# atsuki-ichikawa/KoeMorph

Measured on AMD Instinct MI355X. Metric: blendshape frames/sec (52-coef, 256-win, d_model=256), higher is better.
Workload: dtype f32; 1 GPU; C2: 256 windows/GPU x 136448 samples (8.5 s @16 kHz) -> 1024-pt STFT, hop 533, 80-bin log-mel (257 frames) -> dual-stream attention d_model=256, 8 heads, window 256 -> 52 coefficients + EMA; from audio resident in HBM (rotating batches); windows_per_gpu=256, samples_per_window=136448, parallelism=window-sharded x1, no collective

## Files before the change

### koemorph_amd/csrc/km_device.h

```cpp
#pragma once

#include <hip/hip_runtime.h>

#include "koemorph.h"

namespace km {

struct LogParams {
    int log_mode;
    float amin, top_db, db_add, db_scale, log_eps;
};

__device__ __forceinline__ float clamp_lo(float x, float lo) { return __builtin_amdgcn_fmed3f(x, lo, __builtin_inff()); }
__device__ __forceinline__ float db10(float s, float amin) {
    return 3.01029995663981195f * __builtin_amdgcn_logf(clamp_lo(s, amin));
}

__device__ __forceinline__ void log_window_consts(const LogParams& p, float ref, float& ref_db, float& floor_db) {
    ref_db = db10(ref, p.amin);
    floor_db = (db10(ref, p.amin) - ref_db) - p.top_db;
}

__device__ __forceinline__ float db_finish(const LogParams& p, float dbs, float ref_db, float floor_db) {
    float v = dbs - ref_db;
    v = clamp_lo(v, floor_db);
    return (v + p.db_add) * p.db_scale;
}
__device__ __forceinline__ float db_fast_c1(const LogParams& p, float ref_db) { return (p.db_add - ref_db) * p.db_scale; }
__device__ __forceinline__ float db_finish_fast(float dbs, float scale, float c1) { return fmaxf(fmaf(dbs, scale, c1), 0.f); }
struct DbXform { LogParams lp; const unsigned* ref_bits; };

struct LnXform { const float* stats; const float* gamma; const float* beta; int npart; float eps; };
__device__ __forceinline__ void ln_combine(const float2* __restrict__ st, int npart, float eps, float& rs, float& nmurs, float* mean_out = nullptr) {
    float msum = 0.f;
    for (int p = 0; p < npart; ++p) msum += st[p].x;
    const float mean = msum / (float)npart;
    float m2 = 0.f;
    for (int p = 0; p < npart; ++p) { const float dm = st[p].x - mean; m2 += st[p].y + 32.0f * dm * dm; }
    rs = 1.0f / sqrtf(m2 / (float)(32 * npart) + eps);
    nmurs = -mean * rs;
    if (mean_out) *mean_out = mean;
}
__device__ __forceinline__ void ln_combine8(const float2 (&st)[8], int npart, float eps, float& rs, float& nmurs) {
    float msum = 0.f;
#pragma unroll
    for (int p = 0; p < 8; ++p) msum += p < npart ? st[p].x : 0.f;
    const float mean = msum / (float)npart;
    float m2 = 0.f;
#pragma unroll
    for (int p = 0; p < 8; ++p) { const float dm = st[p].x - mean; m2 += p < npart ? st[p].y + 32.0f * dm * dm : 0.f; }
    rs = 1.0f / sqrtf(m2 / (float)(32 * npart) + eps);
    nmurs = -mean * rs;
}
__device__ __forceinline__ float ln_apply(float x, float rs, float nmurs, float gam, float bet) { return fmaf(fmaf(x, rs, nmurs), gam, bet); }

template <int MODE>
__device__ __forceinline__ float log_one_t(const LogParams& p, float s, float ref_db, float floor_db) {
    if (MODE == KM_LOG_LN_EPS) return 0.693147180559945309f * __builtin_amdgcn_logf(s + p.log_eps);
    float v = db10(s, p.amin) - ref_db;
    v = clamp_lo(v, floor_db);
    return (v + p.db_add) * p.db_scale;
}

__device__ __forceinline__ float log_one(const LogParams& p, float s, float ref_db, float floor_db) {
    return p.log_mode == KM_LOG_LN_EPS ? log_one_t<KM_LOG_LN_EPS>(p, s, ref_db, floor_db)
                                       : log_one_t<KM_LOG_DB_MAX>(p, s, ref_db, floor_db);
}

template <int MODE>
__device__ __forceinline__ float4 log_four_t(const LogParams& p, float4 v, float ref_db, float floor_db) {
    return make_float4(log_one_t<MODE>(p, v.x, ref_db, floor_db), log_one_t<MODE>(p, v.y, ref_db, floor_db),
                       log_one_t<MODE>(p, v.z, ref_db, floor_db), log_one_t<MODE>(p, v.w, ref_db, floor_db));
}

__device__ __forceinline__ float row16_sum(float v) {
    v += __int_as_float(__builtin_amdgcn_update_dpp(0, __float_as_int(v), 0xB1, 0xF, 0xF, true));
    v += __int_as_float(__builtin_amdgcn_update_dpp(0, __float_as_int(v), 0x4E, 0xF, 0xF, true));
    v += __int_as_float(__builtin_amdgcn_update_dpp(0, __float_as_int(v), 0x141, 0xF, 0xF, true));
    v += __int_as_float(__builtin_amdgcn_update_dpp(0, __float_as_int(v), 0x140, 0xF, 0xF, true));
    return v;
}

struct EmoArgs {
    const float* emo = nullptr;
    int ED = 0;
    const float *wee_t = nullptr , *bee = nullptr, *lg = nullptr, *lb = nullptr, *we2 = nullptr, *be2 = nullptr,
                *w2 = nullptr, *b2 = nullptr;
    float* zemo = nullptr;
    int d = 256, DH = 128;
};

__device__ __forceinline__ void emotion_window_d256(const EmoArgs& e, int64_t b, float* scratch) {
    constexpr int d = 256, DH = 128;
    float* emo_s = scratch;
    float* e1 = scratch + 256;
    float* part = scratch + 512;
    const int tid = threadIdx.x, lane = tid & 63;
    if (tid < 256) emo_s[tid] = tid < e.ED ? e.emo[b * e.ED + tid] : 0.f;
    __syncthreads();
    {
        const int n = tid & 255, h = __builtin_amdgcn_readfirstlane(tid >> 8);
#pragma unroll 1
        for (int q = 2 * h; q < 2 * h + 2; ++q) {
            const float* wp = e.wee_t + (size_t)64 * q * d + n;
            float w[64];
#pragma unroll
            for (int u = 0; u < 64; ++u) w[u] = wp[u * d];
            float acc = 0.f;
#pragma unroll
            for (int u = 0; u < 64; u += 4) {
                const float4 x = *reinterpret_cast<const float4*>(emo_s + 64 * q + u);
                acc = fmaf(x.x, w[u], acc);
                acc = fmaf(x.y, w[u + 1], acc);
                acc = fmaf(x.z, w[u + 2], acc);
                acc = fmaf(x.w, w[u + 3], acc);
            }
            part[q * d + n] = acc;
        }
    }
    __syncthreads();
    if (tid < 256) {
        float s = e.bee[tid];
#pragma unroll
        for (int q = 0; q < 4; ++q) s += part[q * d + tid];
        e1[tid] = s;
    }
    __syncthreads();
    if (tid < 64) {
        float x[4], s = 0.f;
#pragma unroll
        for (int i = 0; i < 4; ++i) { x[i] = e1[lane + 64 * i]; s += x[i]; }
#pragma unroll
        for (int o = 32; o > 0; o >>= 1) s += __shfl_xor(s, o);
        const float mean = s * (1.0f / d);
        float v = 0.f;
#pragma unroll
        for (int i = 0; i < 4; ++i) { const float t = x[i] - mean; v += t * t; }
#pragma unroll
        for (int o = 32; o > 0; o >>= 1) v += __shfl_xor(v, o);
        const float rstd = 1.0f / sqrtf(v * (1.0f / d) + 1e-5f);
#pragma unroll
        for (int i = 0; i < 4; ++i) {
            const int c = lane + 64 * i;
            e1[c] = (x[i] - mean) * rstd * e.lg[c] + e.lb[c];
        }
    }
    __syncthreads();
    {
        const int m = tid & 127, h = tid >> 7;
#pragma unroll 1
        for (int q = 2 * h; q < 2 * h + 2; ++q) {
            const float* wp = e.we2 + (size_t)32 * q * DH + m;
            float w[32];
#pragma unroll
            for (int u = 0; u < 32; ++u) w[u] = wp[u * DH];
            float acc = 0.f;
#pragma unroll
            for (int u = 0; u < 32; u += 4) {
                const float4 x = *reinterpret_cast<const float4*>(e1 + 32 * q + u);
                acc = fmaf(x.x, w[u], acc);
                acc = fmaf(x.y, w[u + 1], acc);
                acc = fmaf(x.z, w[u + 2], acc);
                acc = fmaf(x.w, w[u + 3], acc);
            }
            part[q * DH + m] = acc;
        }
    }
    __syncthreads();
    if (tid < 64) {
        float s = 0.f;
#pragma unroll
        for (int i = 0; i < 2; ++i) {
            const int mm = lane + 64 * i;
            float hsum = e.be2[mm];
#pragma unroll
            for (int q = 0; q < 8; ++q) hsum += part[q * DH + mm];
            s += fmaxf(hsum, 0.f) * e.w2[mm];
        }
#pragma unroll
        for (int o = 32; o > 0; o >>= 1) s += __shfl_xor(s, o);
        if (lane == 0) e.zemo[b] = s + e.b2[0];
    }
    __syncthreads();
}

struct EmoShape { int d = 0, DH = 0; };

__device__ __forceinline__ void emotion_layer_f4(const float* __restrict__ w, int K, int N, const float* x, float* part) {
    const int tid = threadIdx.x;
    const int tpr = N >> 2;
    const int G = 512 / tpr;
    const int c4 = tid & (tpr - 1), g = tid / tpr;
    const int kc = (K + G - 1) / G;
    const int k0 = g * kc, k1 = (k0 + kc) < K ? (k0 + kc) : K;
    float4 acc = make_float4(0.f, 0.f, 0.f, 0.f);
    const float* wp = w + 4 * c4;
    for (int k = k0; k < k1; k += 16) {
        float4 wv[16];
#pragma unroll
        for (int u = 0; u < 16; ++u) wv[u] = (k + u) < k1 ? *reinterpret_cast<const float4*>(wp + (size_t)(k + u) * N) : make_float4(0.f, 0.f, 0.f, 0.f);
#pragma unroll
        for (int u = 0; u < 16; ++u) {
            const float xv = (k + u) < k1 ? x[k + u] : 0.f;
            acc.x = fmaf(xv, wv[u].x, acc.x); acc.y = fmaf(xv, wv[u].y, acc.y);
            acc.z = fmaf(xv, wv[u].z, acc.z); acc.w = fmaf(xv, wv[u].w, acc.w);
        }
    }
    *reinterpret_cast<float4*>(part + g * N + 4 * c4) = acc;
}

__device__ __forceinline__ void emotion_window_generic(const EmoArgs& e, const EmoShape sh, int64_t b, float* scratch) {
    const int d = sh.d, DH = sh.DH;
    float* emo_s = scratch;
    float* e1 = scratch + 256;
    float* part = e1 + d;
    const int tid = threadIdx.x, lane = tid & 63;
    if (tid < 256) emo_s[tid] = tid < e.ED ? e.emo[b * e.ED + tid] : 0.f;
    __syncthreads();
    emotion_layer_f4(e.wee_t, e.ED, d, emo_s, part);
    __syncthreads();
    {
        const int G1 = 2048 / d;
        for (int n = tid; n < d; n += 512) {
            float s = e.bee[n];
            for (int g = 0; g < G1; ++g) s += part[g * d + n];
            e1[n] = s;
        }
    }
    __syncthreads();
    if (tid < 64) {
        float s = 0.f;
        for (int n = lane; n < d; n += 64) s += e1[n];
#pragma unroll
        for (int o = 32; o > 0; o >>= 1) s += __shfl_xor(s, o);
        const float mean = s / d;
        float v = 0.f;
        for (int n = lane; n < d; n += 64) { const float t = e1[n] - mean; v += t * t; }
#pragma unroll
        for (int o = 32; o > 0; o >>= 1) v += __shfl_xor(v, o);
        const float rstd = 1.0f / sqrtf(v / d + 1e-5f);
        for (int n = lane; n < d; n += 64) e1[n] = (e1[n] - mean) * rstd * e.lg[n] + e.lb[n];
    }
    __syncthreads();
    emotion_layer_f4(e.we2, d, DH, e1, part);
    __syncthreads();
    if (tid < 64) {
        const int G2 = 2048 / DH;
        float s = 0.f;
        for (int m = lane; m < DH; m += 64) {
            float h = e.be2[m];
            for (int g = 0; g < G2; ++g) h += part[g * DH + m];
            s += fmaxf(h, 0.f) * e.w2[m];
        }
#pragma unroll
        for (int o = 32; o > 0; o >>= 1) s += __shfl_xor(s, o);
        if (lane == 0) e.zemo[b] = s + e.b2[0];
    }
    __syncthreads();
}

}
```

### koemorph_amd/csrc/km_mel.hip

```cpp
#include <hip/hip_runtime.h>

#include <cstdlib>

#include "km_context.h"
#include "km_device.h"

namespace km {

#define HIP_TRY(expr)                                                                         \
    do {                                                                                      \
        hipError_t e_ = (expr);                                                               \
        if (e_ != hipSuccess) return fail(KM_ERR_HIP, "%s: %s", #expr, hipGetErrorString(e_)); \
    } while (0)

namespace mel {
constexpr int FPB = 16;
constexpr int WAVES = 4;
constexpr int FFT_BUF = 1152;
}

__device__ __forceinline__ float2 cadd(float2 a, float2 b) { return make_float2(a.x + b.x, a.y + b.y); }
__device__ __forceinline__ float2 csub(float2 a, float2 b) { return make_float2(a.x - b.x, a.y - b.y); }
__device__ __forceinline__ float2 cmul(float2 a, float2 b) {
    return make_float2(a.x * b.x - a.y * b.y, a.x * b.y + a.y * b.x);
// ... 430 lines not shown
#define KM_MEL_W2 0
#endif
__device__ __forceinline__ void swap_lane32(v2f& a, v2f& b) {
    const auto r0 = __builtin_amdgcn_permlane32_swap(__float_as_uint(a.x), __float_as_uint(b.x), false, false);
    const auto r1 = __builtin_amdgcn_permlane32_swap(__float_as_uint(a.y), __float_as_uint(b.y), false, false);
    a = v2f{__uint_as_float(r0[0]), __uint_as_float(r1[0])}; b = v2f{__uint_as_float(r0[1]), __uint_as_float(r1[1])};
}
__device__ __forceinline__ void swap_lane16(v2f& a, v2f& b) {
    const auto r0 = __builtin_amdgcn_permlane16_swap(__float_as_uint(a.x), __float_as_uint(b.x), false, false);
    const auto r1 = __builtin_amdgcn_permlane16_swap(__float_as_uint(a.y), __float_as_uint(b.y), false, false);
    a = v2f{__uint_as_float(r0[0]), __uint_as_float(r1[0])}; b = v2f{__uint_as_float(r0[1]), __uint_as_float(r1[1])};
}
#define KM_XM " row_mask:0xf bank_mask:"
#define KM_XBANK(CT, MT, CA, MA, MB)                                      \
    "s_nop 1\n\t"                                                        \
    "v_mov_b32_dpp %[t0], %[a0] " CT KM_XM MT "\n\t"                      \
    "v_mov_b32_dpp %[t1], %[a1] " CT KM_XM MT "\n\t"                      \
    "v_mov_b32_dpp %[t2], %[a2] " CT KM_XM MT "\n\t"                      \
    "v_mov_b32_dpp %[t3], %[a3] " CT KM_XM MT "\n\t"                      \
    "v_mov_b32_dpp %[a0], %[b0] " CA KM_XM MA "\n\t"                      \
    "v_mov_b32_dpp %[a1], %[b1] " CA KM_XM MA "\n\t"                      \
    "v_mov_b32_dpp %[a2], %[b2] " CA KM_XM MA "\n\t"                      \
    "v_mov_b32_dpp %[a3], %[b3] " CA KM_XM MA "\n\t"                      \
    "v_mov_b32_dpp %[b0], %[t0] quad_perm:[0,1,2,3]" KM_XM MB "\n\t"      \
    "v_mov_b32_dpp %[b1], %[t1] quad_perm:[0,1,2,3]" KM_XM MB "\n\t"      \
    "v_mov_b32_dpp %[b2], %[t2] quad_perm:[0,1,2,3]" KM_XM MB "\n\t"      \
    "v_mov_b32_dpp %[b3], %[t3] quad_perm:[0,1,2,3]" KM_XM MB "\n\t"      \
    "s_nop 0"
#define KM_XBANK_OPERANDS                                                                                              \
    : [t0] "=&v"(t0), [t1] "=&v"(t1), [t2] "=&v"(t2), [t3] "=&v"(t3), [a0] "+v"(p0), [a1] "+v"(p1), [a2] "+v"(p2), [a3] "+v"(p3), \
      [b0] "+v"(q0), [b1] "+v"(q1), [b2] "+v"(q2), [b3] "+v"(q3)
#define KM_XQUAD(QP)                                                       \
    "s_nop 1\n\t"                                                          \
    "v_mov_b32_dpp %[t0], %[a0] " QP KM_XM "0xf\n\t"                        \
    "v_mov_b32_dpp %[t1], %[a1] " QP KM_XM "0xf\n\t"                        \
    "v_mov_b32_dpp %[u0], %[b0] " QP KM_XM "0xf\n\t"                        \
    "v_mov_b32_dpp %[u1], %[b1] " QP KM_XM "0xf\n\t"                        \
    "v_mov_b32_dpp %[t2], %[a2] " QP KM_XM "0xf\n\t"                        \
    "v_mov_b32_dpp %[t3], %[a3] " QP KM_XM "0xf\n\t"                        \
    "v_mov_b32_dpp %[u2], %[b2] " QP KM_XM "0xf\n\t"                        \
    "v_mov_b32_dpp %[u3], %[b3] " QP KM_XM "0xf\n\t"                        \
    "v_cndmask_b32_e64 %[a0], %[a0], %[u0], %[mk]\n\t"                      \
    "v_cndmask_b32_e64 %[a1], %[a1], %[u1], %[mk]\n\t"                      \
    "v_cndmask_b32_e64 %[b0], %[t0], %[b0], %[mk]\n\t"                      \
    "v_cndmask_b32_e64 %[b1], %[t1], %[b1], %[mk]\n\t"                      \
    "v_cndmask_b32_e64 %[a2], %[a2], %[u2], %[mk]\n\t"                      \
    "v_cndmask_b32_e64 %[a3], %[a3], %[u3], %[mk]\n\t"                      \
    "v_cndmask_b32_e64 %[b2], %[t2], %[b2], %[mk]\n\t"                      \
    "v_cndmask_b32_e64 %[b3], %[t3], %[b3], %[mk]\n\t"                      \
    "s_nop 0"
#define KM_XQUAD_OPERANDS                                                                                              \
    : [t0] "=&v"(t0), [t1] "=&v"(t1), [t2] "=&v"(t2), [t3] "=&v"(t3), [u0] "=&v"(u0), [u1] "=&v"(u1), [u2] "=&v"(u2), [u3] "=&v"(u3), \
      [a0] "+v"(p0), [a1] "+v"(p1), [a2] "+v"(p2), [a3] "+v"(p3), [b0] "+v"(q0), [b1] "+v"(q1), [b2] "+v"(q2), [b3] "+v"(q3)       \
    : [mk] "s"(mk)
template <int B>
__device__ __forceinline__ void swap_lane_dpp(v2f& a0, v2f& b0, v2f& a1, v2f& b1) {
    float p0 = a0.x, p1 = a0.y, p2 = a1.x, p3 = a1.y, q0 = b0.x, q1 = b0.y, q2 = b1.x, q3 = b1.y, t0, t1, t2, t3;
    if constexpr (B == 3) KM_ASM(KM_XBANK("row_ror:8", "0xf", "row_ror:8", "0xc", "0x3") KM_XBANK_OPERANDS);
    else if constexpr (B == 2) KM_ASM(KM_XBANK("row_shl:4", "0x5", "row_shr:4", "0xa", "0x5") KM_XBANK_OPERANDS);
    else {
        constexpr unsigned long long mk = B == 1 ? 0xCCCCCCCCCCCCCCCCull : 0xAAAAAAAAAAAAAAAAull;
        float u0, u1, u2, u3;
        if constexpr (B == 1) KM_ASM(KM_XQUAD("quad_perm:[2,3,0,1]") KM_XQUAD_OPERANDS);
        else KM_ASM(KM_XQUAD("quad_perm:[1,0,3,2]") KM_XQUAD_OPERANDS);
    }
    a0 = v2f{p0, p1}; a1 = v2f{p2, p3}; b0 = v2f{q0, q1}; b1 = v2f{q2, q3};
}
__device__ __forceinline__ void exchange_hi(v2f (&y)[8]) {
#pragma unroll
    for (int r = 0; r < 4; ++r) swap_lane32(y[r], y[r + 4]);
#pragma unroll
    for (int r = 0; r < 8; r += 4) { swap_lane16(y[r], y[r + 2]); swap_lane16(y[r + 1], y[r + 3]); }
    swap_lane_dpp<3>(y[0], y[1], y[2], y[3]);
    swap_lane_dpp<3>(y[4], y[5], y[6], y[7]);
}
__device__ __forceinline__ void exchange_lo(v2f (&y)[8]) {
    swap_lane_dpp<2>(y[0], y[4], y[1], y[5]);
    swap_lane_dpp<2>(y[2], y[6], y[3], y[7]);
    swap_lane_dpp<1>(y[0], y[2], y[1], y[3]);
    swap_lane_dpp<1>(y[4], y[6], y[5], y[7]);
    swap_lane_dpp<0>(y[0], y[1], y[2], y[3]);
    swap_lane_dpp<0>(y[4], y[5], y[6], y[7]);
}
__host__ __device__ constexpr int fft_lane_k0(int lane) { return (KM_MEL_XCHG & 1) ? bitrev(lane >> 3, 3) : lane >> 3; }
__host__ __device__ constexpr int fft_lane_bin(int lane) {
    return (KM_MEL_XCHG & 2) ? fft_lane_k0(lane) + 8 * bitrev(lane & 7, 3) : lane;
}
__host__ __device__ constexpr int fft_bin_lane(int c) {
    return (KM_MEL_XCHG & 2) ? 8 * ((KM_MEL_XCHG & 1) ? bitrev(c & 7, 3) : (c & 7)) + bitrev(c >> 3, 3) : c;
}
}

template <bool RING>
__device__ __forceinline__ bool load_frame_rp_fast(const float* __restrict__ x, int Li, int rs, int hop, int f, int lane,
                                                   melrp::v2f (&z)[8]) {
    const int lo = f * hop - 512;
    if (lo < 0 || lo + 1024 > Li) return false;
    int start = lo;
    if constexpr (RING) {
        start += rs;
        start -= start >= Li ? Li : 0;
        if (start + 1024 > Li) return false;
    }
    const float* xp = x + start + 2 * lane;
#pragma unroll
    for (int i = 0; i < 8; ++i) z[i] = melrp::v2f{xp[128 * i], xp[128 * i + 1]};
    return true;
}

__device__ __noinline__ void load_frame_rp_slow(const float* __restrict__ x, int Li, int rs, int ring, int hop, int refl, int f,
                                                int lane, float2* __restrict__ buf) {
    const int p0 = f * hop - 512 + 2 * lane;
    for (int i = 0; i < 8; ++i) {
        float v[2];
        for (int e = 0; e < 2; ++e) {
            int q = p0 + 128 * i + e;
            bool ok = true;
            if (refl) q = q < 0 ? -q : (q >= Li ? 2 * (Li - 1) - q : q);
            else ok = q >= 0 && q < Li;
            if (ring) { q += rs; q -= q >= Li ? Li : 0; }
            v[e] = ok ? x[ok ? q : 0] : 0.f;
        }
        buf[lane + 64 * i] = make_float2(v[0], v[1]);
    }
}

__device__ __forceinline__ int mel_slot_of_lane(int lane) {
    const int m = lane & 31;
    const bool g0 = m < 4 || (m >= 12 && m < 16) || (m >= 20 && m < 28);
    return 2 * (lane >> 5) + (g0 ? 0 : 1);
}
__device__ __forceinline__ int mel_frame_of_lane(int lane) {
    const int m = lane & 31;
    if (m < 4) return m;
    if (m < 12) return m - 4;
    if (m < 16) return m - 8;
    if (m < 20) return m - 8;
    if (m < 28) return m - 12;
    return m - 16;
}
__device__ __forceinline__ int mel_lane_of(int slot, int frame) {
    int m;
    if (slot & 1) m = frame < 8 ? frame + 4 : (frame < 12 ? frame + 8 : frame + 16);
    else m = frame < 4 ? frame : (frame < 8 ? frame + 8 : frame + 12);
    return 32 * (slot >> 1) + m;
}

template <bool RING, bool PACK = false>
__global__ __launch_bounds__(512, 4) void mel_power_rp_kernel(MelArgs a) {
    using namespace melrp;
    extern __shared__ __attribute__((aligned(16))) float smem[];
    float2* fbuf = reinterpret_cast<float2*>(smem);
    float* pw = smem + WAVES * FFT_BUF * 2;
    float* redmax = pw + FPB * NFS;
    int* sched = reinterpret_cast<int*>(redmax + WAVES);
    float* fbw = redmax + WAVES + 4;

#ifdef KM_MEL_STAMP
    const unsigned long long st_entry = __builtin_readcyclecounter(), st_entry_rt = __builtin_amdgcn_s_memrealtime();
#endif
    const int tid = threadIdx.x, lane = tid & 63;
    const int wave = __builtin_amdgcn_readfirstlane(tid >> 6);
#if KM_MEL_REMAP
    const unsigned lin_ = blockIdx.x + gridDim.x * blockIdx.y;
    const int b = (int)(lin_ % gridDim.y), bx = (int)(lin_ / gridDim.y);
#else
    const int b = blockIdx.y, bx = (int)blockIdx.x;
#endif
    const int64_t gw = a.win0 + b;
    const int64_t clip = gw / a.wins_per_clip, woff = (gw - clip * a.wins_per_clip) * a.win_step;
    const float* x = a.audio + clip * a.clip_len + woff;
    const int Lv = (int)((a.clip_len - woff) < a.L ? (a.clip_len - woff) : a.L);
    if (a.ready && !a.ready[b]) return;
    const int rs = RING ? a.ring_start[b] : -1;
    v2f* buf = reinterpret_cast<v2f*>(fbuf + wave * FFT_BUF);
    const int n_chunks = (a.n_frames + FPB - 1) / FPB;
    const unsigned rd2 = lds_offset(buf + (lane >> 3) * 72 + (lane & 7)), rd3 = lds_offset(buf + lane * 9);
    const unsigned wr3 = lds_offset(buf + fft_lane_k0(lane) * 9 + (lane & 7));
    const int cbin = fft_lane_bin(lane);

    v2f zn[8];
    bool zn_ok = false;
    const int fmul = a.frame_mul;
    auto first_frame = [&]() {
        if (KM_MEL_SKIP & 8) {
#pragma unroll
            for (int i = 0; i < 8; ++i) zn[i] = v2f{0.001f * lane, 0.5f + i};
            zn_ok = true;
        } else if (bx * FPB + wave < a.n_frames) zn_ok = load_frame_rp_fast<RING>(x, Lv, rs, a.hop, (bx * FPB + wave) * fmul, lane, zn);
    };
    if (!(KM_MEL_SKIP & 16) && a.emo.emo && bx == (int)gridDim.x - 1) {
        if (a.emo.d == 256 && a.emo.DH == 128) emotion_window_d256(a.emo, gw, pw);
        else emotion_window_generic(a.emo, EmoShape{a.emo.d, a.emo.DH}, gw, pw);
        first_frame();
    } else {
        first_frame();
    }

    const unsigned ctr_last = (unsigned)n_chunks - 1u;
    for (int i = tid; i < a.fbg_nw; i += NT) fbw[i] = a.fbg_weight[i];
    for (int i = tid; i < FPB * (NFS - 513); i += NT) pw[(i / (NFS - 513)) * NFS + 513 + i % (NFS - 513)] = 0.f;

    const int n2 = lane & 7, k0 = fft_lane_k0(lane);
    v2f win2[8], tw1[8], tw2[8], twp[4];
#pragma unroll
    for (int i = 0; i < 8; ++i) {
        win2[i] = v2f{a.window[2 * (lane + 64 * i)], a.window[2 * (lane + 64 * i) + 1]};
        tw1[i] = ld2(a.twiddle + ((2 * lane * bitrev(i, 3)) & 1023));
        tw2[i] = ld2(a.twiddle + ((16 * n2 * bitrev(i, 3)) & 1023));
    }
#pragma unroll
    for (int i = 0; i < 4; ++i) twp[i] = ld2(a.twiddle + cbin + 64 * i);

    int my_gid[NGW];
#pragma unroll
    for (int i = 0; i < NGW; ++i) my_gid[i] = __builtin_amdgcn_readfirstlane(a.fbg_gid[wave * NGW + i]);
    const int* my_desc_p = a.fbg_desc + wave * NGW * 4 + mel_slot_of_lane(lane);
#pragma unroll
    for (int i = 0; i < 8; ++i) asm volatile("" ::"v"(win2[i]), "v"(tw1[i]), "v"(tw2[i]));
#pragma unroll
    for (int i = 0; i < 4; ++i) asm volatile("" ::"v"(twp[i]));
#pragma unroll
    for (int i = 0; i < NGW; ++i) asm volatile("" ::"s"(my_gid[i]));

    float vmax = 0.f;
    int chunk = bx, chunk_next = bx + (int)gridDim.x;
#if defined(KM_MEL_DELAY)
    if (bx & 1) { for (int i = 0; i < KM_MEL_DELAY; i += 16) __builtin_amdgcn_s_sleep(16); }
#endif
#ifdef KM_MEL_STAMP
    unsigned st_acc[16] = {0};
    unsigned long long st_last = __builtin_readcyclecounter();
    const unsigned long long st_first = st_last;
#endif
    while (chunk < n_chunks) {
        unsigned req = 0;
        if (tid == 0) req = atomicAdd(a.chunk_ctr + b, 1u);
        const int f0 = chunk * FPB;
#pragma unroll 1
        for (int pi = 0; pi < FPB / WAVES; ++pi) {
            const int fl = wave + WAVES * pi;
            const int f = f0 + fl;
            if (f < a.n_frames) {
                if (!zn_ok) {
                    load_frame_rp_slow(x, Lv, rs, RING ? 1 : 0, a.hop, a.pad_mode == KM_PAD_REFLECT ? 1 : 0, f * fmul, lane,
                                       reinterpret_cast<float2*>(buf));
                    __builtin_amdgcn_wave_barrier();
#pragma unroll
                    for (int i = 0; i < 8; ++i) zn[i] = buf[lane + 64 * i];
                    __builtin_amdgcn_wave_barrier();
                }
                KM_STAMP(0);
                v2f z[8];
#pragma unroll
                for (int i = 0; i < 8; ++i) z[i] = zn[i] * win2[i];
                if (!(KM_MEL_SKIP & 4)) { dif8(z); cmul7(z, tw1); }
                KM_STAMP(1);
                v2f y[8];
                if ((KM_MEL_XCHG & 1) && !(KM_MEL_SKIP & 2)) {
                    exchange_hi(z);
#pragma unroll
                    for (int i = 0; i < 8; ++i) y[i] = z[i];
                } else if (!(KM_MEL_SKIP & 2)) {
#pragma unroll
                    for (int i = 0; i < 8; ++i) buf[bitrev(i, 3) * 72 + lane] = z[i];
                    __builtin_amdgcn_wave_barrier();
                }
                {
                    const int fnext = pi + 1 < FPB / WAVES ? f + WAVES : chunk_next * FPB + wave;
                    if (!(KM_MEL_SKIP & 8)) zn_ok = fnext < a.n_frames && load_frame_rp_fast<RING>(x, Lv, rs, a.hop, fnext * fmul, lane, zn);
                }
                if (!(KM_MEL_XCHG & 1) && !(KM_MEL_SKIP & 2)) {
                    lds_read8<64>(rd2, y);
                    __builtin_amdgcn_wave_barrier();
                } else if (KM_MEL_SKIP & 2) {
#pragma unroll
                    for (int i = 0; i < 8; ++i) y[i] = z[i];
                }
                KM_STAMP(2);
                if (!(KM_MEL_SKIP & 4)) { dif8(y); cmul7(y, tw2); }
                KM_STAMP(3);
                if ((KM_MEL_XCHG & 2) && !(KM_MEL_SKIP & 2)) {
                    exchange_lo(y);
                } else if (!(KM_MEL_SKIP & 2)) {
#if KM_MEL_W2
#pragma unroll
                    for (int i = 0; i < 8; ++i) buf[(k0 + 8 * bitrev(i, 3)) * 9 + n2] = y[i];
#else
                    lds_write8_bitrev<8 * 9 * 8>(wr3, y);
#endif
                    __builtin_amdgcn_wave_barrier();
                    lds_read8<8>(rd3, y);
                    __builtin_amdgcn_wave_barrier();
                }
                KM_STAMP(4);
                if (!(KM_MEL_SKIP & 4)) dif8(y);
                KM_STAMP(5);
                float* pwr = pw + fl * NFS;
                v2f zk[4], zc[4];
                v2f zmid = y[1];
                if (!(KM_MEL_SKIP & 2)) {
                    const int src = fft_bin_lane((64 - cbin) & 63) << 2;
                    auto perm = [&](v2f v) {
                        return v2f{__int_as_float(__builtin_amdgcn_ds_bpermute(src, __float_as_int(v.x))),
                                   __int_as_float(__builtin_amdgcn_ds_bpermute(src, __float_as_int(v.y)))};
                    };
                    const v2f p7 = perm(y[7]), p3 = perm(y[3]), p5 = perm(y[5]), p1 = perm(y[1]);
                    const bool l0 = lane == 0;
                    zk[0] = y[0]; zk[1] = y[4]; zk[2] = y[2]; zk[3] = y[6];
                    zc[0] = l0 ? y[0] : p7; zc[1] = l0 ? y[7] : p3; zc[2] = l0 ? y[3] : p5; zc[3] = l0 ? y[5] : p1;
                } else {
#pragma unroll
                    for (int i = 0; i < 4; ++i) { zk[i] = y[i]; zc[i] = y[i + 4]; }
                }
                KM_STAMP(6);
                if (!(KM_MEL_SKIP & 4)) post4(zk, zc, twp);
#pragma unroll
                for (int i = 0; i < 4; ++i) {
                    pwr[cbin + 64 * i] = zk[i].x;
                    pwr[2 * 256 - cbin - 64 * i] = zk[i].y;
                }
                if (lane == 0) pwr[256] = 4.0f * (zmid.x * zmid.x + zmid.y * zmid.y);
                KM_STAMP(7);
            }
        }
        KM_STAMP(8);
        int my_desc[NGW];
#pragma unroll
        for (int i = 0; i < NGW; ++i) my_desc[i] = my_desc_p[4 * i];
        if (tid == 0) {
            if (req == ctr_last) a.chunk_ctr[b] = 0u;
            sched[0] = (int)(req + 2u * gridDim.x);
        }
        __syncthreads();
        KM_STAMP(9);
        if (KM_MEL_PRIO) __builtin_amdgcn_s_setprio(KM_MEL_PRIO);
        {
            const int slot = mel_slot_of_lane(lane), flm = mel_frame_of_lane(lane);
            const bool fvalid = f0 + flm < a.n_frames;
            const float4* prow = reinterpret_cast<const float4*>(pw + flm * NFS);
            const float4* wbase = reinterpret_cast<const float4*>(fbw);
            float* dst = a.melpow + ((int64_t)b * a.n_frames + f0 + flm) * a.n_mels + slot;
            const int fr = f0 + flm, qs = a.n_frames >= 3 ? fr - (a.n_frames - 3) : fr;
            const bool st_long = fvalid && fr < a.pack_T, st_short = fvalid && qs >= 0 && qs < 3;
            float* dst_long = nullptr; float* dst_short = nullptr;
            if constexpr (PACK) {
                dst_long = a.pack_xt + ((int64_t)b * a.n_mels + slot) * a.pack_KP + fr;
                dst_short = a.pack_xt + ((int64_t)b * a.n_mels + slot) * a.pack_KP + a.pack_T + qs;
            }
            auto store_mel = [&](int gid, float r) {
                if (4 * gid + slot >= a.n_mels) return;
                if constexpr (PACK) {
                    const float db = db10(r, a.pack_amin);
                    if (st_long) dst_long[(int64_t)4 * gid * a.pack_KP] = db;
                    if (st_short) dst_short[(int64_t)4 * gid * a.pack_KP] = db;
                } else {
                    if (fvalid) dst[4 * gid] = r;
                }
            };
            float fmx = 0.f;
#if KM_MEL_FLAT
            auto group_pr = [&](int i) { return prow + (my_desc[i] & 255); };
            auto group_wt = [&](int i) { return wbase + ((unsigned)my_desc[i] >> 16); };
            float4 wv = make_float4(0.f, 0.f, 0.f, 0.f), pv = wv;
            if (!(KM_MEL_SKIP & 1) && my_gid[0] >= 0) { wv = group_wt(0)[0]; pv = group_pr(0)[0]; }
#pragma unroll
            for (int i = 0; i < ((KM_MEL_SKIP & 1) ? 0 : NGW); ++i) {
                if (my_gid[i] < 0) break;
                const int steps = __builtin_amdgcn_readfirstlane((my_desc[i] >> 8) & 255);
                const float4* pr = group_pr(i);
                const float4* wt = group_wt(i);
                v2f acc = {0.f, 0.f};
                for (int t = 1; t < steps; ++t) {
                    const float4 wn = wt[t], pn = pr[t];
                    acc = __builtin_elementwise_fma(v2f{pv.x, pv.y}, v2f{wv.x, wv.y}, acc);
                    acc = __builtin_elementwise_fma(v2f{pv.z, pv.w}, v2f{wv.z, wv.w}, acc);
                    pv = pn; wv = wn;
                }
                float4 wn = wv, pn = pv;
                if (i + 1 < NGW && my_gid[i + 1 < NGW ? i + 1 : i] >= 0) { wn = group_wt(i + 1 < NGW ? i + 1 : i)[0]; pn = group_pr(i + 1 < NGW ? i + 1 : i)[0]; }
                acc = __builtin_elementwise_fma(v2f{pv.x, pv.y}, v2f{wv.x, wv.y}, acc);
                acc = __builtin_elementwise_fma(v2f{pv.z, pv.w}, v2f{wv.z, wv.w}, acc);
                pv = pn; wv = wn;
                float r = acc.x + acc.y;
                r = fvalid ? r : 0.f;
                asm("v_max_f32 %0, %0, %1" : "+v"(vmax) : "v"(r));
                asm("v_max_f32 %0, %0, %1" : "+v"(fmx) : "v"(r));
                store_mel(my_gid[i], r);
            }
#else
#pragma unroll
            for (int i = 0; i < ((KM_MEL_SKIP & 1) ? 0 : NGW); ++i) {
                if (my_gid[i] < 0) break;
                const int desc = my_desc[i];
                const int steps = __builtin_amdgcn_readfirstlane((desc >> 8) & 255);
                const float4* pr = prow + (desc & 255);
                const float4* wt = wbase + ((unsigned)desc >> 16);
                v2f acc = {0.f, 0.f};
                float4 wv = wt[0], pv = pr[0];
                for (int t = 1; t < steps; ++t) {
                    const float4 wn = wt[t], pn = pr[t];
                    acc = __builtin_elementwise_fma(v2f{pv.x, pv.y}, v2f{wv.x, wv.y}, acc);
                    acc = __builtin_elementwise_fma(v2f{pv.z, pv.w}, v2f{wv.z, wv.w}, acc);
                    pv = pn; wv = wn;
                }
                acc = __builtin_elementwise_fma(v2f{pv.x, pv.y}, v2f{wv.x, wv.y}, acc);
                acc = __builtin_elementwise_fma(v2f{pv.z, pv.w}, v2f{wv.z, wv.w}, acc);
                float r = acc.x + acc.y;
                r = fvalid ? r : 0.f;
                asm("v_max_f32 %0, %0, %1" : "+v"(vmax) : "v"(r));
                asm("v_max_f32 %0, %0, %1" : "+v"(fmx) : "v"(r));
                store_mel(my_gid[i], r);
            }
#endif
            if (a.frame_max) {
                float fall = fmx;
#pragma unroll
                for (int s2 = 0; s2 < 4; ++s2) fall = fmaxf(fall, __shfl(fmx, mel_lane_of(s2, flm)));
                fmx = fall;
                if (slot == 0 && fvalid) atomicMax(a.frame_max + (int64_t)b * a.n_frames + f0 + flm, __float_as_uint(fmx));
            }
        }
        if (KM_MEL_PRIO) __builtin_amdgcn_s_setprio(0);
        KM_STAMP(10);
        chunk = chunk_next;
        chunk_next = __builtin_amdgcn_readfirstlane(sched[0]);
        __syncthreads();
        KM_STAMP(11);
    }
#ifdef KM_MEL_STAMP
    if (lane == 0) {
        unsigned long long* o = km_mel_stamps + ((size_t)(b * gridDim.x + bx) * WAVES + wave) * 24;
        if (b * gridDim.x + bx < 1024) {
            for (int i = 0; i < 12; ++i) o[i] = st_acc[i];
            o[12] = st_last - st_first;
            o[13] = st_entry; o[14] = st_first; o[15] = st_last; o[16] = st_entry_rt; o[17] = __builtin_amdgcn_s_memrealtime();
            o[18] = __builtin_readcyclecounter();
        }
    }
#endif
#pragma unroll
    for (int o = 32; o > 0; o >>= 1) vmax = fmaxf(vmax, __shfl_xor(vmax, o));
    if (lane == 0) redmax[wave] = vmax;
    __syncthreads();
    if (tid == 0 && !a.frame_max) {
        float mx = redmax[0];
#pragma unroll
        for (int w = 1; w < WAVES; ++w) mx = fmaxf(mx, redmax[w]);
        atomicMax(a.melmax + b, __float_as_uint(mx));
    }
}

struct LogArgs {
    const float* melpow;
    const unsigned* melmax;
    int n_frames, out_frames, n_mels;
    LogParams lp;
    float* mel_long;
    float* mel_short;
};

__global__ __launch_bounds__(256) void mel_log_kernel(LogArgs a) {
    const int b = blockIdx.y;
    float ref_db, floor_db;
    log_window_consts(a.lp, __uint_as_float(a.melmax[b]), ref_db, floor_db);
    const float* src = a.melpow + (int64_t)b * a.n_frames * a.n_mels;
    const int total = a.out_frames * a.n_mels;
    const int i = blockIdx.x * 256 + threadIdx.x;
    if (i < total) {
        int f = i / a.n_mels;
        const int m = i - f * a.n_mels;
        if (f >= a.n_frames) f = a.n_frames - 1;
        a.mel_long[(int64_t)b * total + i] = log_one(a.lp, src[f * a.n_mels + m], ref_db, floor_db);
    }
    if (a.mel_short && blockIdx.x == 0) {
        for (int s = threadIdx.x; s < 3 * a.n_mels; s += 256) {
            const int r = s / a.n_mels, m = s - r * a.n_mels;
            float v = 0.f;
            if (a.n_frames >= 3) v = log_one(a.lp, src[(a.n_frames - 3 + r) * a.n_mels + m], ref_db, floor_db);
            else if (r < a.n_frames) v = log_one(a.lp, src[r * a.n_mels + m], ref_db, floor_db);
            a.mel_short[(int64_t)b * 3 * a.n_mels + s] = v;
        }
    }
}

__global__ __launch_bounds__(256) void mel_log_packed_kernel(LogArgs a, float* __restrict__ xp, int T, int KP) {
    const int b = blockIdx.y;
    float ref_db, floor_db;
    log_window_consts(a.lp, __uint_as_float(a.melmax[b]), ref_db, floor_db);
    const float* src = a.melpow + (int64_t)b * a.n_frames * a.n_mels;
    const int i = blockIdx.x * 256 + threadIdx.x;
    if (i >= KP * a.n_mels) return;
    const int r = i / a.n_mels, m = i - r * a.n_mels;
    int f = -1;
    if (r < T) f = r < a.n_frames ? r : -1;
    else if (r < T + 3) {
        const int q = r - T;
        if (a.n_frames >= 3) f = a.n_frames - 3 + q; else if (q < a.n_frames) f = q;
    }
    xp[(int64_t)b * KP * a.n_mels + i] = f >= 0 ? log_one(a.lp, src[f * a.n_mels + m], ref_db, floor_db) : 0.f;
}

template <typename Tv>
static int upload(Tv** dst, const std::vector<Tv>& src) {
    HIP_TRY(hipMalloc(reinterpret_cast<void**>(dst), src.size() * sizeof(Tv)));
    HIP_TRY(hipMemcpy(*dst, src.data(), src.size() * sizeof(Tv), hipMemcpyHostToDevice));
    return KM_OK;
}

int upload_mel_plan(MelPlan* p) {
    if (p->uploaded) return KM_OK;
    if (int rc = upload(&p->d_window, p->window)) return rc;
    if (int rc = upload(&p->d_twiddle, p->twiddle)) return rc;
    if (int rc = upload(&p->d_fb_start, p->fb_start)) return rc;
    if (int rc = upload(&p->d_fb_count, p->fb_count)) return rc;
    if (int rc = upload(&p->d_fb_offset, p->fb_offset)) return rc;
    if (int rc = upload(&p->d_fb_weight, p->fb_weight)) return rc;
    if (!p->fbg_gid.empty()) {
        if (int rc = upload(&p->d_fbg_gid, p->fbg_gid)) return rc;
        if (int rc = upload(&p->d_fbg_desc, p->fbg_desc)) return rc;
        if (int rc = upload(&p->d_fbg_weight, p->fbg_weight)) return rc;
    }
    p->uploaded = true;
    return KM_OK;
}
// ... 218 lines not shown
```

Before: 1.842 million frames/s.

## Replace shuffles with swizzle/permlane reductions, DPP FFT mirror, optional tiled emotion MLP

Wave reductions that used __shfl_xor now go through ds_swizzle, with permlane32_swap for the 32-lane step. The default FFT lane-to-bin mapping becomes a permutation whose mirror partners sit within one DPP row, so the conjugate-bin exchange uses a DPP row_mirror instead of ds_bpermute. The per-frame max reduction is shortened to two xor steps. A batched emotion MLP path that processes several windows per block is added behind KM_EMO_TILE, which defaults to 1 and leaves the old per-window path in place. The new lane mapping changes LDS read addresses and bin order, which risks correctness or bank conflicts if the mirror mapping is wrong.

```diff
diff --git a/koemorph_amd/csrc/km_device.h b/koemorph_amd/csrc/km_device.h
--- a/koemorph_amd/csrc/km_device.h
+++ b/koemorph_amd/csrc/km_device.h
@@ -90,6 +90,157 @@
     int d = 256, DH = 128;
 };
 
+template <int O>
+__device__ __forceinline__ float xor_lane(float v) {
+    static_assert(O > 0 && O < 64 && (O & (O - 1)) == 0, "xor distance");
+    if constexpr (O == 32) {
+        const auto r = __builtin_amdgcn_permlane32_swap(__float_as_uint(v), __float_as_uint(v), false, false);
+        return __uint_as_float((threadIdx.x & 32) ? r[0] : r[1]);
+    } else {
+        return __int_as_float(__builtin_amdgcn_ds_swizzle(__float_as_int(v), (O << 10) | 0x1F));
+    }
+}
+__device__ __forceinline__ float wave_sum_xor(float s) {
+    s += xor_lane<32>(s); s += xor_lane<16>(s); s += xor_lane<8>(s);
+    s += xor_lane<4>(s); s += xor_lane<2>(s); s += xor_lane<1>(s);
+    return s;
+}
+
+#ifndef KM_EMO_TILE
+#define KM_EMO_TILE 1
+#endif
+constexpr int kEmoTile = KM_EMO_TILE, kEmoTileScratch = 256 * kEmoTile + 7 * 128 * kEmoTile;
+__device__ __forceinline__ void emotion_tile_d256(const EmoArgs& e, int64_t g0, int n, const unsigned char* ready, float* scratch) {
+    constexpr int d = 256, DH = 128, TW = kEmoTile > 1 ? kEmoTile : 4;
+    static_assert(TW % 4 == 0 && TW <= 16, "tile width (KM_EMO_TILE 1: emotion_window_d256)");
+    typedef float v2 __attribute__((ext_vector_type(2)));
+    float* xt = scratch;
+    float* s1 = scratch + d * TW;
+    float* p1 = s1 + d * TW;
+    const int tid = threadIdx.x, lane = tid & 63, wave = tid >> 6;
+    for (int i = tid; i < d * TW; i += 512) {
+        const int w = i >> 8, k = i & 255;
+        xt[k * TW + w] = (w < n && k < e.ED) ? e.emo[(g0 + w) * e.ED + k] : 0.f;
+    }
+    __syncthreads();
+    {
+        const int c = tid & 255, h = __builtin_amdgcn_readfirstlane(tid >> 8);
+#pragma unroll 1
+        for (int q = 2 * h; q < 2 * h + 2; ++q) {
+            const float* wp = e.wee_t + (size_t)64 * q * d + c;
+            float w[64];
+#pragma unroll
+            for (int u = 0; u < 64; ++u) w[u] = wp[u * d];
+            v2 acc[TW / 2];
+#pragma unroll
+            for (int j = 0; j < TW / 2; ++j) acc[j] = v2{0.f, 0.f};
+#pragma unroll
+            for (int u = 0; u < 64; ++u) {
+                const float* xr = xt + (64 * q + u) * TW;
+#pragma unroll
+                for (int j = 0; j < TW / 4; ++j) {
+                    const float4 x = *reinterpret_cast<const float4*>(xr + 4 * j);
+                    acc[2 * j] = __builtin_elementwise_fma(v2{x.x, x.y}, v2{w[u], w[u]}, acc[2 * j]);
+                    acc[2 * j + 1] = __builtin_elementwise_fma(v2{x.z, x.w}, v2{w[u], w[u]}, acc[2 * j + 1]);
+                }
+            }
+            if (q == 0) {
+                const float b = e.bee[c];
+#pragma unroll
+                for (int j = 0; j < TW / 2; ++j) { s1[(2 * j) * d + c] = b + acc[j].x; s1[(2 * j + 1) * d + c] = b + acc[j].y; }
+            } else if (q == 1) {
+#pragma unroll
+                for (int j = 0; j < TW / 2; ++j) { s1[(2 * j) * d + c] += acc[j].x; s1[(2 * j + 1) * d + c] += acc[j].y; }
+            } else {
+                float* pq = p1 + (q - 2) * TW * d;
+#pragma unroll
+                for (int j = 0; j < TW / 2; ++j) { pq[(2 * j) * d + c] = acc[j].x; pq[(2 * j + 1) * d + c] = acc[j].y; }
+            }
+        }
+    }
+    __syncthreads();
+    for (int i = tid; i < TW * d; i += 512) {
+        float s = s1[i];
+        s += p1[i];
+        s += p1[TW * d + i];
+        s1[i] = s;
+    }
+    __syncthreads();
+#pragma unroll 1
+    for (int w = wave; w < TW; w += 8) {
+        const float* e1 = s1 + w * d;
+        float x[4], s = 0.f;
+#pragma unroll
+        for (int i = 0; i < 4; ++i) { x[i] = e1[lane + 64 * i]; s += x[i]; }
+        s = wave_sum_xor(s);
+        const float mean = s * (1.0f / d);
+        float v = 0.f;
+#pragma unroll
+        for (int i = 0; i < 4; ++i) { const float t = x[i] - mean; v += t * t; }
+        v = wave_sum_xor(v);
+        const float rstd = 1.0f / sqrtf(v * (1.0f / d) + 1e-5f);
+#pragma unroll
+        for (int i = 0; i < 4; ++i) {
+            const int c = lane + 64 * i;
+            xt[c * TW + w] = (x[i] - mean) * rstd * e.lg[c] + e.lb[c];
+        }
+    }
+    __syncthreads();
+    float* s2 = s1;
+    float* p2 = s1 + DH * TW;
+    {
+        const int m = tid & 127, h = tid >> 7;
+#pragma unroll 1
+        for (int q = 2 * h; q < 2 * h + 2; ++q) {
+            const float* wp = e.we2 + (size_t)32 * q * DH + m;
+            float w[32];
+#pragma unroll
+            for (int u = 0; u < 32; ++u) w[u] = wp[u * DH];
+            v2 acc[TW / 2];
+#pragma unroll
+            for (int j = 0; j < TW / 2; ++j) acc[j] = v2{0.f, 0.f};
+#pragma unroll
+            for (int u = 0; u < 32; ++u) {
+                const float* xr = xt + (32 * q + u) * TW;
+#pragma unroll
+                for (int j = 0; j < TW / 4; ++j) {
+                    const float4 x = *reinterpret_cast<const float4*>(xr + 4 * j);
+                    acc[2 * j] = __builtin_elementwise_fma(v2{x.x, x.y}, v2{w[u], w[u]}, acc[2 * j]);
+                    acc[2 * j + 1] = __builtin_elementwise_fma(v2{x.z, x.w}, v2{w[u], w[u]}, acc[2 * j + 1]);
+                }
+            }
+            if (q == 0) {
+                const float b = e.be2[m];
+#pragma unroll
+                for (int j = 0; j < TW / 2; ++j) { s2[(2 * j) * DH + m] = b + acc[j].x; s2[(2 * j + 1) * DH + m] = b + acc[j].y; }
+            } else if (q == 1) {
+#pragma unroll
+                for (int j = 0; j < TW / 2; ++j) { s2[(2 * j) * DH + m] += acc[j].x; s2[(2 * j + 1) * DH + m] += acc[j].y; }
+            } else {
+                float* pq = p2 + (q - 2) * TW * DH;
+#pragma unroll
+                for (int j = 0; j < TW / 2; ++j) { pq[(2 * j) * DH + m] = acc[j].x; pq[(2 * j + 1) * DH + m] = acc[j].y; }
+            }
+        }
+    }
+    __syncthreads();
+#pragma unroll 1
+    for (int w = wave; w < TW; w += 8) {
+        float s = 0.f;
+#pragma unroll
+        for (int i = 0; i < 2; ++i) {
+            const int mm = lane + 64 * i;
+            float hsum = s2[w * DH + mm];
+#pragma unroll
+            for (int q = 0; q < 6; ++q) hsum += p2[(q * TW + w) * DH + mm];
+            s += fmaxf(hsum, 0.f) * e.w2[mm];
+        }
+        s = wave_sum_xor(s);
+        if (lane == 0 && w < n && (!ready || ready[w])) e.zemo[g0 + w] = s + e.b2[0];
+    }
+    __syncthreads();
+}
+
 __device__ __forceinline__ void emotion_window_d256(const EmoArgs& e, int64_t b, float* scratch) {
     constexpr int d = 256, DH = 128;
     float* emo_s = scratch;
@@ -130,14 +281,12 @@
         float x[4], s = 0.f;
 #pragma unroll
         for (int i = 0; i < 4; ++i) { x[i] = e1[lane + 64 * i]; s += x[i]; }
-#pragma unroll
-        for (int o = 32; o > 0; o >>= 1) s += __shfl_xor(s, o);
+        s = wave_sum_xor(s);
         const float mean = s * (1.0f / d);
         float v = 0.f;
 #pragma unroll
         for (int i = 0; i < 4; ++i) { const float t = x[i] - mean; v += t * t; }
-#pragma unroll
-        for (int o = 32; o > 0; o >>= 1) v += __shfl_xor(v, o);
+        v = wave_sum_xor(v);
         const float rstd = 1.0f / sqrtf(v * (1.0f / d) + 1e-5f);
 #pragma unroll
         for (int i = 0; i < 4; ++i) {
@@ -177,8 +326,7 @@
             for (int q = 0; q < 8; ++q) hsum += part[q * DH + mm];
             s += fmaxf(hsum, 0.f) * e.w2[mm];
         }
-#pragma unroll
-        for (int o = 32; o > 0; o >>= 1) s += __shfl_xor(s, o);
+        s = wave_sum_xor(s);
         if (lane == 0) e.zemo[b] = s + e.b2[0];
     }
     __syncthreads();
@@ -231,13 +379,11 @@
     if (tid < 64) {
         float s = 0.f;
         for (int n = lane; n < d; n += 64) s += e1[n];
-#pragma unroll
-        for (int o = 32; o > 0; o >>= 1) s += __shfl_xor(s, o);
+        s = wave_sum_xor(s);
         const float mean = s / d;
         float v = 0.f;
         for (int n = lane; n < d; n += 64) { const float t = e1[n] - mean; v += t * t; }
-#pragma unroll
-        for (int o = 32; o > 0; o >>= 1) v += __shfl_xor(v, o);
+        v = wave_sum_xor(v);
         const float rstd = 1.0f / sqrtf(v / d + 1e-5f);
         for (int n = lane; n < d; n += 64) e1[n] = (e1[n] - mean) * rstd * e.lg[n] + e.lb[n];
     }
@@ -252,8 +398,7 @@
             for (int g = 0; g < G2; ++g) h += part[g * DH + m];
             s += fmaxf(h, 0.f) * e.w2[m];
         }
-#pragma unroll
-        for (int o = 32; o > 0; o >>= 1) s += __shfl_xor(s, o);
+        s = wave_sum_xor(s);
         if (lane == 0) e.zemo[b] = s + e.b2[0];
     }
     __syncthreads();
diff --git a/koemorph_amd/csrc/km_mel.hip b/koemorph_amd/csrc/km_mel.hip
--- a/koemorph_amd/csrc/km_mel.hip
+++ b/koemorph_amd/csrc/km_mel.hip
@@ -536,13 +536,27 @@
     swap_lane_dpp<0>(y[0], y[1], y[2], y[3]);
     swap_lane_dpp<0>(y[4], y[5], y[6], y[7]);
 }
+__host__ __device__ constexpr int fft_sigma(int lane) {
+    return (lane & 8) ? (lane == 15 ? 32 : (64 - (8 * (lane >> 4) + (15 - (lane & 15)))) & 63) : 8 * (lane >> 4) + (lane & 7);
+}
+__host__ __device__ constexpr int fft_sigma_inv(int c) {
+    return c == 32 ? 15 : (c <= 32 ? 16 * (c >> 3) + (c & 7) : (16 * ((64 - c) >> 3) + ((64 - c) & 7)) ^ 15);
+}
 __host__ __device__ constexpr int fft_lane_k0(int lane) { return (KM_MEL_XCHG & 1) ? bitrev(lane >> 3, 3) : lane >> 3; }
 __host__ __device__ constexpr int fft_lane_bin(int lane) {
-    return (KM_MEL_XCHG & 2) ? fft_lane_k0(lane) + 8 * bitrev(lane & 7, 3) : lane;
+    return (KM_MEL_XCHG & 2) ? fft_lane_k0(lane) + 8 * bitrev(lane & 7, 3) : fft_sigma(lane);
 }
 __host__ __device__ constexpr int fft_bin_lane(int c) {
-    return (KM_MEL_XCHG & 2) ? 8 * ((KM_MEL_XCHG & 1) ? bitrev(c & 7, 3) : (c & 7)) + bitrev(c >> 3, 3) : c;
-}
+    return (KM_MEL_XCHG & 2) ? 8 * ((KM_MEL_XCHG & 1) ? bitrev(c & 7, 3) : (c & 7)) + bitrev(c >> 3, 3) : fft_sigma_inv(c);
+}
+constexpr bool fft_sigma_ok() {
+    for (int l = 0; l < 64; ++l) {
+        if (fft_sigma_inv(fft_sigma(l)) != l) return false;
+        if (l != 0 && l != 15 && fft_sigma(l ^ 15) != ((64 - fft_sigma(l)) & 63)) return false;
+    }
+    return fft_sigma(0) == 0 && fft_sigma(15) == 32;
+}
+static_assert(fft_sigma_ok(), "fft_sigma: a permutation with mirror partners");
 }
 
 template <bool RING>
@@ -625,13 +639,20 @@
     const int64_t clip = gw / a.wins_per_clip, woff = (gw - clip * a.wins_per_clip) * a.win_step;
     const float* x = a.audio + clip * a.clip_len + woff;
     const int Lv = (int)((a.clip_len - woff) < a.L ? (a.clip_len - woff) : a.L);
+    const bool emo_rider = !(KM_MEL_SKIP & 16) && a.emo.emo && bx == (int)gridDim.x - 1;
+    const bool emo_tile = a.emo.d == 256 && a.emo.DH == 128;
+    static_assert(WAVES * FFT_BUF * 2 + FPB * NFS >= kEmoTileScratch, "emotion tile scratch");
+    if (kEmoTile > 1 && emo_rider && emo_tile && b % kEmoTile == 0) {
+        const int n = (int)gridDim.y - b < kEmoTile ? (int)gridDim.y - b : kEmoTile;
+        emotion_tile_d256(a.emo, gw, n, a.ready ? a.ready + b : nullptr, smem);
+    }
     if (a.ready && !a.ready[b]) return;
     const int rs = RING ? a.ring_start[b] : -1;
     v2f* buf = reinterpret_cast<v2f*>(fbuf + wave * FFT_BUF);
     const int n_chunks = (a.n_frames + FPB - 1) / FPB;
-    const unsigned rd2 = lds_offset(buf + (lane >> 3) * 72 + (lane & 7)), rd3 = lds_offset(buf + lane * 9);
+    const int cbin = fft_lane_bin(lane);
+    const unsigned rd2 = lds_offset(buf + (lane >> 3) * 72 + (lane & 7)), rd3 = lds_offset(buf + cbin * 9);
     const unsigned wr3 = lds_offset(buf + fft_lane_k0(lane) * 9 + (lane & 7));
-    const int cbin = fft_lane_bin(lane);
 
     v2f zn[8];
     bool zn_ok = false;
@@ -643,13 +664,9 @@
             zn_ok = true;
         } else if (bx * FPB + wave < a.n_frames) zn_ok = load_frame_rp_fast<RING>(x, Lv, rs, a.hop, (bx * FPB + wave) * fmul, lane, zn);
     };
-    if (!(KM_MEL_SKIP & 16) && a.emo.emo && bx == (int)gridDim.x - 1) {
-        if (a.emo.d == 256 && a.emo.DH == 128) emotion_window_d256(a.emo, gw, pw);
-        else emotion_window_generic(a.emo, EmoShape{a.emo.d, a.emo.DH}, gw, pw);
-        first_frame();
-    } else {
-        first_frame();
-    }
+    if (kEmoTile == 1 && emo_rider && emo_tile) emotion_window_d256(a.emo, gw, pw);
+    if (emo_rider && !emo_tile) emotion_window_generic(a.emo, EmoShape{a.emo.d, a.emo.DH}, gw, pw);
+    first_frame();
 
     const unsigned ctr_last = (unsigned)n_chunks - 1u;
     for (int i = tid; i < a.fbg_nw; i += NT) fbw[i] = a.fbg_weight[i];
@@ -753,6 +770,19 @@
                 float* pwr = pw + fl * NFS;
                 v2f zk[4], zc[4];
                 v2f zmid = y[1];
+#if !(KM_MEL_XCHG & 2)
+                if (!(KM_MEL_SKIP & 2)) {
+                    auto mirror = [](v2f v) {
+                        return v2f{__int_as_float(__builtin_amdgcn_update_dpp(0, __float_as_int(v.x), 0x140, 0xF, 0xF, true)),
+                                   __int_as_float(__builtin_amdgcn_update_dpp(0, __float_as_int(v.y), 0x140, 0xF, 0xF, true))};
+                    };
+                    const v2f p7 = mirror(y[7]), p3 = mirror(y[3]), p5 = mirror(y[5]), p1 = mirror(y[1]);
+                    const bool l0 = lane == 0, l15 = lane == 15;
+                    zk[0] = y[0]; zk[1] = y[4]; zk[2] = y[2]; zk[3] = y[6];
+                    zc[0] = l0 ? y[0] : (l15 ? y[7] : p7); zc[1] = l0 ? y[7] : (l15 ? y[3] : p3);
+                    zc[2] = l0 ? y[3] : (l15 ? y[5] : p5); zc[3] = l0 ? y[5] : (l15 ? y[1] : p1);
+                }
+#else
                 if (!(KM_MEL_SKIP & 2)) {
                     const int src = fft_bin_lane((64 - cbin) & 63) << 2;
                     auto perm = [&](v2f v) {
@@ -763,7 +793,9 @@
                     const bool l0 = lane == 0;
                     zk[0] = y[0]; zk[1] = y[4]; zk[2] = y[2]; zk[3] = y[6];
                     zc[0] = l0 ? y[0] : p7; zc[1] = l0 ? y[7] : p3; zc[2] = l0 ? y[3] : p5; zc[3] = l0 ? y[5] : p1;
-                } else {
+                }
+#endif
+                else {
 #pragma unroll
                     for (int i = 0; i < 4; ++i) { zk[i] = y[i]; zc[i] = y[i + 4]; }
                 }
@@ -868,10 +900,8 @@
             }
 #endif
             if (a.frame_max) {
-                float fall = fmx;
-#pragma unroll
-                for (int s2 = 0; s2 < 4; ++s2) fall = fmaxf(fall, __shfl(fmx, mel_lane_of(s2, flm)));
-                fmx = fall;
+                const float f2 = fmaxf(fmx, xor_lane<4>(fmx));
+                fmx = fmaxf(f2, xor_lane<32>(f2));
                 if (slot == 0 && fvalid) atomicMax(a.frame_max + (int64_t)b * a.n_frames + f0 + flm, __float_as_uint(fmx));
             }
         }
@@ -893,8 +923,8 @@
         }
     }
 #endif
-#pragma unroll
-    for (int o = 32; o > 0; o >>= 1) vmax = fmaxf(vmax, __shfl_xor(vmax, o));
+    vmax = fmaxf(vmax, xor_lane<32>(vmax)); vmax = fmaxf(vmax, xor_lane<16>(vmax)); vmax = fmaxf(vmax, xor_lane<8>(vmax));
+    vmax = fmaxf(vmax, xor_lane<4>(vmax)); vmax = fmaxf(vmax, xor_lane<2>(vmax)); vmax = fmaxf(vmax, xor_lane<1>(vmax));
     if (lane == 0) redmax[wave] = vmax;
     __syncthreads();
     if (tid == 0 && !a.frame_max) {
```

Result: faster. 1.872 million frames/s, median of 6 (+1.6%).
